# MSU-dcypherlab/mfgp-coverage

Measured on NVIDIA B200. Metric: GP posterior mean+var + coverage step, grid-points/s (coverage iterations/s = 1000/ms_per_step), higher is better.
Workload: dtype f64

## Files before the change

### mfgp-coverage_b200/csrc/common.cuh

```cuda
#pragma once
#include <cstdint>
#include <cstdio>
#include <cuda_runtime.h>

#include "../../include/mfgp_b200.h"

namespace mfgp {

void set_last_error(const char* what, cudaError_t e);

#define MFGP_CUDA_CHECK(expr)                                   \
    do {                                                        \
        cudaError_t _e = (expr);                                \
        if (_e != cudaSuccess) {                                \
            ::mfgp::set_last_error(#expr, _e);                  \
            return MFGP_ERR_CUDA;                               \
        }                                                       \
    } while (0)

void count_launch();
#define MFGP_LAUNCH_CHECK()                  \
    do {                                     \
        ::mfgp::count_launch();              \
        MFGP_CUDA_CHECK(cudaGetLastError()); \
    } while (0)

__device__ __forceinline__ void dmma884(double& c0, double& c1, double a, double b) {
    asm volatile("mma.sync.aligned.m8n8k4.row.col.f64.f64.f64.f64 {%0,%1}, {%2}, {%3}, {%0,%1};\n"
                 : "+d"(c0), "+d"(c1)
                 : "d"(a), "d"(b));
}

__device__ __forceinline__ void cp_async16(void* smem_dst, const void* gmem_src, bool valid) {
    unsigned s = static_cast<unsigned>(__cvta_generic_to_shared(smem_dst));
    int bytes = valid ? 16 : 0;
    asm volatile("cp.async.cg.shared.global [%0], [%1], 16, %2;\n" ::"r"(s), "l"(gmem_src), "r"(bytes));
}
__device__ __forceinline__ void cp_async_commit() { asm volatile("cp.async.commit_group;\n" ::); }
template <int N>
__device__ __forceinline__ void cp_async_wait() {
    asm volatile("cp.async.wait_group %0;\n" ::"n"(N));
}

__device__ __forceinline__ double rbf_scaled(double ax, double ay, double bx, double by, double scale) {
    double d0 = ax - bx, d1 = ay - by;
    double q = __dadd_rn(__dmul_rn(d0, d0), __dmul_rn(d1, d1));
    return scale * exp(-0.5 * q);
}

struct DevParams {
    double s_L, inv_unused, s_H, rho, rho2, noise_L, noise_H, mean_L, mean_H, jitter, l_L, l_H, k0;
    int multi;
};

inline DevParams make_dev_params(const mfgp_params& p) {
    DevParams d;
    d.s_L = p.multi ? p.s_L : 0.0;
    d.inv_unused = 0.0;
    d.s_H = p.s_H;
    d.rho = p.multi ? p.rho : 1.0;
    d.rho2 = d.rho * d.rho;
    d.noise_L = p.noise_L;
    d.noise_H = p.noise_H;
    d.mean_L = p.mean_L;
    d.mean_H = p.mean_H;
    d.jitter = p.jitter;
// ... 9 lines not shown
```

### mfgp-coverage_b200/csrc/gp_fit.cu

```cuda
#include "common.cuh"
#include "gemm_f64.cuh"
#include <cstdlib>
#include <cstring>

namespace mfgp {

__global__ void scaled_coords_kernel(const double* __restrict__ Xt, int N, int npad, DevParams p, double* __restrict__ Tt) {
    const int i = blockIdx.x * blockDim.x + threadIdx.x;
    if (i >= npad) return;
    double4 t = make_double4(0.0, 0.0, 0.0, 0.0);
    if (i < N) {
        const double xi = Xt[2 * i], yi = Xt[2 * i + 1];
        t = make_double4(xi / p.l_L, yi / p.l_L, xi / p.l_H, yi / p.l_H);
    }
    reinterpret_cast<double4*>(Tt)[i] = t;
}

__global__ void build_train_cov_kernel(const double* __restrict__ Xt, int NL, int NH, DevParams p, double* __restrict__ K,
                                       int npad, int64_t ld, const double* __restrict__ Tt, int row_begin) {
    const int j = blockIdx.x * blockDim.x + threadIdx.x;
    const int i = row_begin + blockIdx.y * blockDim.y + threadIdx.y;
    const int N = NL + NH;
    if (i >= npad || j >= npad) return;
    if (j >= ((i >> 6) + 1) * 64) return;
// ... 22 lines not shown
                const double kH = rbf_scaled(a.z, a.w, b.z, b.w, p.s_H);
                v = __dadd_rn(__dmul_rn(p.rho2, kL), kH);
                if (i == j) v = v + p.noise_H;
            }
        } else {
            v = rbf_scaled(a.z, a.w, b.z, b.w, p.s_H);
            if (i == j) v = v + p.noise_H;
        }
        if (i == j) v = v + p.jitter;
    }
    K[(int64_t)i * ld + j] = v;
}

constexpr int PB = 64;
constexpr int PLD = PB + 1;

struct PotrfScratch {
    double2 colAB[2][PB], rowAB[2][PB];
    double piv[3][PB / 2];
    double fin[3][PB / 2];
    int bad;
};

template <int BS>
__device__ __forceinline__ void potrf_diag_body(const double* src, int64_t lds, double* A, int64_t ld,
                                                double* __restrict__ Winv, int64_t ldw, int32_t* __restrict__ info, int col0,
                                                PotrfScratch* sc, double* Lsm = nullptr, double* Wsm = nullptr, int lds_out = 0) {
    constexpr int NB = BS / 16;
    double2 (*colAB)[PB] = sc->colAB;
    double2 (*rowAB)[PB] = sc->rowAB;
    double (*piv)[PB / 2] = sc->piv;
    double (*fin)[PB / 2] = sc->fin;
    int& bad = sc->bad;
    const int tid = threadIdx.x;
    const int ti = tid >> 4, tc = tid & 15;
    if (tid == 0) bad = 0;
    double s[NB][NB], m[NB][NB];
#pragma unroll
    for (int a = 0; a < NB; a++)
#pragma unroll
        for (int b = 0; b < NB; b++) {
            const int r = ti + 16 * a, c = tc + 16 * b;
            s[a][b] = (c <= r) ? src[(int64_t)r * lds + c] : 0.0;
            m[a][b] = (r == c) ? 1.0 : 0.0;
        }
#pragma unroll
    for (int jb = 0; jb < NB; jb++) {
#pragma unroll 1
        for (int jp = 0; jp < 8; jp++) {
            const int k = jb * 8 + jp, j0 = 2 * k, j1 = j0 + 1, jj0 = 2 * jp, buf = k & 1;
            if ((tc & 14) == jj0) {
                double* dst = reinterpret_cast<double*>(colAB[buf]) + (tc & 1);
#pragma unroll
                for (int a = 0; a < NB; a++) dst[2 * (ti + 16 * a)] = s[a][jb];
            }
            if ((ti & 14) == jj0) {
                double* dst = reinterpret_cast<double*>(rowAB[buf]) + (ti & 1);
#pragma unroll
                for (int b = 0; b < NB; b++) dst[2 * (tc + 16 * b)] = m[jb][b];
            }
            __syncthreads();
            const double2* col = colAB[buf];
            const double2* row = rowAB[buf];
            double pa = col[j0].x;
            const double2 p1 = col[j1];
            double pb = p1.x, pc = p1.y;
            double det = fma(pa, pc, -(pb * pb));
            if (!(pa > 0.0) || !(det > 0.0)) {
                if (tid == 0 && !bad) {
                    bad = 1;
                    atomicCAS(info, 0, col0 + ((pa > 0.0) ? j1 : j0) + 1);
                }
                pa = 1.0; pb = 0.0; pc = 1.0; det = 1.0;
            }
            if (tid == 0) { piv[0][k] = pa; piv[1][k] = pb; piv[2][k] = pc; }
            const double idet = 1.0 / det;
            const double qa = pc * idet, qb = -pb * idet, qc = pa * idet;
            double t1[NB], t2[NB];
#pragma unroll
            for (int a = 0; a < NB; a++) {
                if (a < jb) continue;
                const double2 x = col[ti + 16 * a];
                t1[a] = fma(qa, x.x, qb * x.y);
                t2[a] = fma(qb, x.x, qc * x.y);
// ... 2 lines not shown
            for (int b = 0; b < NB; b++) {
                if (b < jb) continue;
                const double2 y = col[tc + 16 * b];
                const bool live = tc + 16 * b > j1;
#pragma unroll
                for (int a = 0; a < NB; a++) {
                    if (a < b) continue;
                    if (live) s[a][b] = fma(-t1[a], y.x, fma(-t2[a], y.y, s[a][b]));
                }
            }
#pragma unroll
            for (int b = 0; b < NB; b++) {
                if (b > jb) continue;
                const double2 z = row[tc + 16 * b];
#pragma unroll
                for (int a = 0; a < NB; a++) {
                    if (a < jb) continue;
                    const bool live = ti + 16 * a > j1;
                    if (live) m[a][b] = fma(-t1[a], z.x, fma(-t2[a], z.y, m[a][b]));
                }
            }
        }
    }
    __syncthreads();
    if (tid < BS / 2) {
        const double a = piv[0][tid], b = piv[1][tid], c = piv[2][tid];
        const double r1 = rsqrt(a);
        const double g = b * r1 * r1;
        fin[0][tid] = r1;
        fin[1][tid] = rsqrt(fma(-g, b, c));
        fin[2][tid] = g;
    }
    __syncthreads();
    const bool failed = bad != 0;
#pragma unroll
    for (int a = 0; a < NB; a++)
#pragma unroll
        for (int b = 0; b < NB; b++) {
            const int r = ti + 16 * a, c = tc + 16 * b;
            const double v = s[a][b], w = m[a][b];
            const double vp = __shfl_up_sync(0xffffffffu, v, 1);
            const double wp = __shfl_up_sync(0xffffffffu, w, 16);
            const int kc = c >> 1, kr = r >> 1;
            const double lv = (c & 1) ? (v - fin[2][kc] * vp) * fin[1][kc] : v * fin[0][kc];
            const double wv = (r & 1) ? (w - fin[2][kr] * wp) * fin[1][kr] : w * fin[0][kr];
            const double lo = failed ? ((r == c) ? 1.0 : 0.0) : ((c <= r) ? lv : 0.0);
            const double wo = failed ? ((r == c) ? 1.0 : 0.0) : ((c <= r) ? wv : 0.0);
            if (c <= r) A[(int64_t)r * ld + c] = lo;
            if (Winv != nullptr) Winv[(int64_t)r * ldw + c] = wo;
            if (Lsm != nullptr) Lsm[r * lds_out + c] = lo;
            if (Wsm != nullptr) Wsm[r * lds_out + c] = wo;
        }
}

__global__ void __launch_bounds__(256, 1) potrf_diag_kernel(double* __restrict__ A, int64_t ld, double* __restrict__ Winv,
                                                         int64_t ldw, int32_t* __restrict__ info, int jblk) {
    __shared__ __align__(16) PotrfScratch scratch;
    potrf_diag_body<PB>(A, ld, A, ld, Winv, ldw, info, jblk * PB, &scratch);
}

constexpr int DF_K = 32;
constexpr int DF_LDA = DF_K + 4;
constexpr int DF_LDT = PB + 4;
constexpr int DF_STAGE = PB * DF_LDA;
constexpr int DF_TILE = PB * DF_LDT;
constexpr int DF_NSTAGE = 3;
constexpr int DF_SMEM_DOUBLES = DF_NSTAGE * 2 * DF_STAGE;
constexpr int DF_THREADS = 256;

struct DfArgs {
    double* K; int64_t ld;
    double* W; int64_t ldw;
    double* Bm; int64_t ldb;
    int nb, nr;
    int32_t* info;
    int* flagsL;
    int* flagsY;
    int* ctrl;
    int* pause;
    int total;
    double* M; int64_t ldm;
    int* flagsM;
    int mg, m_full, m_tiles, m_total, m_lead;
    long long spin_limit;
    long long* trace;
    int chain_la;
};

__host__ __device__ __forceinline__ void df_group_rows(int gi, int nb, int mg, int m_full, int& kb, int& ke) {
    if (gi < m_full) { kb = gi * mg; ke = kb + mg; return; }
    kb = m_full * mg;
// ... 13 lines not shown

__device__ __forceinline__ void df_stamp(long long* trace, int task, int k) {
    if (trace != nullptr && threadIdx.x == 0) {
        unsigned long long t;
        asm volatile("mov.u64 %0, %%globaltimer;\n" : "=l"(t));
        trace[task * 16 + k] = (long long)t;
        trace[task * 16 + 8 + k] = clock64();
    }
}

__device__ __forceinline__ int df_ld_acquire(const int* p) {
    int v;
    asm volatile("ld.acquire.gpu.global.s32 %0, [%1];\n" : "=r"(v) : "l"(p) : "memory");
    return v;
}
__device__ __forceinline__ int df_ld_relaxed(const int* p) {
    int v;
    asm volatile("ld.relaxed.gpu.global.s32 %0, [%1];\n" : "=r"(v) : "l"(p) : "memory");
    return v;
}
__device__ __forceinline__ void df_st_release(int* p, int v) {
    asm volatile("st.release.gpu.global.s32 [%0], %1;\n" ::"l"(p), "r"(v) : "memory");
}
__device__ __forceinline__ void df_st_relaxed(int* p, int v) {
    asm volatile("st.relaxed.gpu.global.s32 [%0], %1;\n" ::"l"(p), "r"(v) : "memory");
}
__device__ __forceinline__ bool df_wait(const int* f, int* ctrl, int32_t* info, long long limit) {
    int ok = 1;
    if ((threadIdx.x & 31) == 0) {
        if (!df_ld_relaxed(f)) {
            const long long t0 = clock64();
            while (!df_ld_relaxed(f)) {
                __nanosleep(32);
                if (clock64() - t0 > limit) { atomicExch(ctrl + 1, 1); atomicExch(info, -1); }
                if (*reinterpret_cast<volatile int*>(ctrl + 1)) { ok = 0; break; }
            }
        }
        (void)df_ld_acquire(f);
    }
    ok = __shfl_sync(0xffffffffu, ok, 0);
    __syncwarp();
    return ok != 0;
}

__global__ void __launch_bounds__(DF_THREADS, 2) chol_dataflow_kernel(DfArgs g) {
    extern __shared__ __align__(16) double df_smem[];
    __shared__ int task[4];
    __shared__ int ready_s[4];
    const int tid = threadIdx.x, lane = tid & 31, warp = tid >> 5;
    const int wm = (warp >> 1) * 8, wn = (warp & 1) * 8;
    const int gq = lane >> 2, tq = lane & 3;
    double* As0 = df_smem;
    double* Bs0 = df_smem + DF_NSTAGE * DF_STAGE;
    unsigned smid;
    asm volatile("mov.u32 %0, %%smid;\n" : "=r"(smid));
    int* my_pause = g.pause + smid;
#ifdef MFGP_DF_ACCOUNTING
    long long t_wait = 0, t_loop = 0, t_begin = clock64(), t_mark = 0;
    int n_tasks = 0;
    const bool tracing = g.trace != nullptr;
#else
    long long t_wait = 0, t_loop = 0, t_begin = 0, t_mark = 0;
    int n_tasks = 0;
    constexpr bool tracing = false;
#endif
    int held_m = -1;
    int dec_c = 0, dec_dnext = 1, dec_base = 1;

    for (;;) {
// ... 506 lines not shown
int side_for_current_device(SideStream** out) {
    int dev = 0;
    MFGP_CUDA_CHECK(cudaGetDevice(&dev));
    if (dev < 0 || dev >= 16) return MFGP_ERR_INVALID;
    SideStream& s = g_side[dev];
    if (!s.st) {
        int least = 0, greatest = 0;
        MFGP_CUDA_CHECK(cudaDeviceGetStreamPriorityRange(&least, &greatest));
        MFGP_CUDA_CHECK(cudaStreamCreateWithPriority(&s.st, cudaStreamNonBlocking, greatest));
        for (int i = 0; i < 2; i++) {
            MFGP_CUDA_CHECK(cudaEventCreateWithFlags(&s.ev_potrf[i], cudaEventDisableTiming));
            MFGP_CUDA_CHECK(cudaEventCreateWithFlags(&s.ev_trsm[i], cudaEventDisableTiming));
        }
        MFGP_CUDA_CHECK(cudaEventCreateWithFlags(&s.ev_begin, cudaEventDisableTiming));
        MFGP_CUDA_CHECK(cudaEventCreateWithFlags(&s.ev_end, cudaEventDisableTiming));
        s.device = dev;
    }
    *out = &s;
    return MFGP_OK;
}
}

namespace {
struct DfScratch {
    long long* trace = nullptr;
    int trace_nb = 0;
    int trace_grid = 0;
    int sms = 0;
};
DfScratch g_df[16];

bool use_panel_chain() {
    static const int v = [] {
        const char* e = getenv("MFGP_CHOL");
        return (e && std::strcmp(e, "chain") == 0) ? 1 : 0;
    }();
    return v != 0;
}

int chol_dataflow(double* K, int64_t npad, int64_t ld, double* W, int64_t ldw, int32_t* info, double* Bm, int64_t ldb, int64_t R,
                  double* M, int64_t ldm, int* scratch, cudaStream_t st) {
    int dev = 0;
    MFGP_CUDA_CHECK(cudaGetDevice(&dev));
    if (dev < 0 || dev >= 16 || !scratch) return MFGP_ERR_INVALID;
    DfScratch& sc = g_df[dev];
    const int nb = (int)(npad / PB), nr = (int)(R / PB);
    const int64_t need = df_scratch_ints(npad, R, M != nullptr);
    if (!sc.sms) MFGP_CUDA_CHECK(cudaDeviceGetAttribute(&sc.sms, cudaDevAttrMultiProcessorCount, dev));
    MFGP_CUDA_CHECK(cudaMemsetAsync(scratch, 0, need * sizeof(int), st));
    MFGP_CUDA_CHECK(cudaMemsetAsync(info, 0, sizeof(int32_t), st));
    DfArgs a{};
    a.K = K; a.ld = ld; a.W = W; a.ldw = ldw; a.Bm = Bm; a.ldb = ldb; a.nb = nb; a.nr = nr; a.info = info;
    a.ctrl = scratch; a.pause = scratch + DF_CTRL_INTS; a.flagsL = a.pause + 1024; a.flagsY = a.flagsL + (int64_t)nb * nb;
    a.total = nb + (nb - 1) * (nb - 2) / 2 + nb * nr;
    if (M != nullptr && nr > 0) {
        static const int mg_env = [] { const char* e = getenv("MFGP_DF_MG"); return e ? atoi(e) : 8; }();
        static const int lead_env = [] { const char* e = getenv("MFGP_DF_MLEAD"); return e ? atoi(e) : 32; }();
        a.M = M; a.ldm = ldm; a.flagsM = a.flagsY + (int64_t)nb * nr;
        a.mg = mg_env < DF_MIN_MG ? DF_MIN_MG : mg_env;
        a.m_tiles = nr * (nr + 1) / 2;
        a.m_total = df_gram_groups(nb, a.mg, a.m_full) * a.m_tiles;
        a.m_lead = lead_env;
    }
    static const bool want_trace = [] { const char* e = getenv("MFGP_DF_TRACE"); return e && atoi(e) != 0; }();
    if (want_trace) {
        if (!sc.trace) MFGP_CUDA_CHECK(cudaMalloc(&sc.trace, 1024 * 24 * sizeof(long long)));
        MFGP_CUDA_CHECK(cudaMemsetAsync(sc.trace, 0, 1024 * 24 * sizeof(long long), st));
        a.trace = nb <= 1024 ? sc.trace : nullptr;
        sc.trace_nb = nb;
    }
    static const int chain_la = [] { const char* e = getenv("MFGP_DF_CHAIN_LA"); return e ? atoi(e) : 5; }();
    a.chain_la = chain_la;
    a.spin_limit = 4000000000LL;
    constexpr int smem = DF_SMEM_DOUBLES * sizeof(double);
    static const int occ = [] { const char* e = getenv("MFGP_DF_OCC"); return e ? atoi(e) : 2; }();
    MFGP_CUDA_CHECK(cudaFuncSetAttribute(chol_dataflow_kernel, cudaFuncAttributeMaxDynamicSharedMemorySize, smem));
    int grid = (occ < 1 ? 1 : occ) * sc.sms;
    if (grid > a.total + a.m_total) grid = a.total + a.m_total;
    sc.trace_grid = grid < 1024 ? grid : 1024;
    chol_dataflow_kernel<<<grid, DF_THREADS, smem, st>>>(a);
    MFGP_LAUNCH_CHECK();
    return MFGP_OK;
}
}

extern "C" int64_t mfgp_debug_chol_trace(int64_t* out, int64_t max_tasks) {
    int dev = 0;
    if (cudaGetDevice(&dev) != cudaSuccess || dev < 0 || dev >= 16) return 0;
    DfScratch& sc = g_df[dev];
    if (!sc.trace || !out) return 0;
    if (max_tasks < 0) {
        if (cudaMemcpy(out, sc.trace + 1024 * 16, 1024 * 8 * sizeof(long long), cudaMemcpyDeviceToHost) != cudaSuccess) return 0;
        return sc.trace_grid;
    }
    int64_t n = sc.trace_nb < max_tasks ? sc.trace_nb : max_tasks;
    if (cudaMemcpy(out, sc.trace, n * 16 * sizeof(long long), cudaMemcpyDeviceToHost) != cudaSuccess) return 0;
    return n;
}

extern "C" int mfgp_cholesky(double* K, int64_t npad, int64_t ld, double* W, int64_t ldw, int32_t* info, void* work,
                             void* stream) {
    if (!K || !info || npad <= 0 || npad % MFGP_TILE || ld < npad) return MFGP_ERR_INVALID;
    if (!W && !work) return MFGP_ERR_INVALID;
// ... 256 lines not shown
```

### mfgp-coverage_b200/csrc/gp_posterior.cu

```cuda
#include <cuda.h>

#include "common.cuh"

namespace mfgp {

constexpr int P_BM = 512;
constexpr int P_BN = 32;
constexpr int P_BK = 16;
constexpr int P_STAGES = 3;
constexpr int P_CONSUMER_WARPS = 8;
constexpr int P_PRODUCER_WARPS = 4;
constexpr int P_THREADS = (P_CONSUMER_WARPS + P_PRODUCER_WARPS) * 32;
constexpr int P_MI = 8;
constexpr int P_NI = 4;
constexpr int P_PLD = P_BK + 4;
constexpr int P_W_STAGE_BYTES = P_BM * P_BK * 8;
constexpr int P_PSI_STAGE_BYTES = P_BN * P_PLD * 8;
constexpr int P_SMEM_BYTES = P_STAGES * (P_W_STAGE_BYTES + P_PSI_STAGE_BYTES) + P_BN * 4 * 8 +
                             P_CONSUMER_WARPS * P_BN * 2 * 8 + 2 * P_STAGES * 8 + 1024 ;

struct PostArgs {
    const double* Xs; int64_t G;
    const double* TLx; const double* TLy; const double* THx; const double* THy;
    int64_t ldt; int64_t g_lo; int ny;
    const double* Tt; int NL, NH;
    int npad;
    const double* z;
    double* mu; double* var; double* qout;
    double* Vc; int64_t ldv;
    int remap_cols;
    int row_lo;
    DevParams p;
};

__device__ __forceinline__ uint32_t smem_u32(const void* p) { return static_cast<uint32_t>(__cvta_generic_to_shared(p)); }
__device__ __forceinline__ void mbar_init(uint32_t bar, uint32_t count) {
    asm volatile("mbarrier.init.shared::cta.b64 [%0], %1;\n" ::"r"(bar), "r"(count));
}
__device__ __forceinline__ void mbar_arrive(uint32_t bar) {
    asm volatile("mbarrier.arrive.shared::cta.b64 _, [%0];\n" ::"r"(bar) : "memory");
}
__device__ __forceinline__ void mbar_expect_tx(uint32_t bar, uint32_t bytes) {
    asm volatile("mbarrier.expect_tx.relaxed.cta.shared::cta.b64 [%0], %1;\n" ::"r"(bar), "r"(bytes) : "memory");
}
__device__ __forceinline__ void mbar_wait(uint32_t bar, uint32_t parity) {
    uint32_t done;
    do {
        asm volatile(
            "{\n .reg .pred p;\n mbarrier.try_wait.parity.shared::cta.b64 p, [%1], %2;\n selp.u32 %0, 1, 0, p;\n}\n"
            : "=r"(done)
            : "r"(bar), "r"(parity)
            : "memory");
    } while (!done);
}
__device__ __forceinline__ void tma_load_2d(uint32_t dst, const CUtensorMap* map, int c0, int c1, uint32_t bar) {
    asm volatile(
        "cp.async.bulk.tensor.2d.shared::cluster.global.mbarrier::complete_tx::bytes [%0], [%1, {%2, %3}], [%4];\n" ::"r"(dst),
        "l"(map), "r"(c0), "r"(c1), "r"(bar)
        : "memory");
}
template <int R>
__device__ __forceinline__ void reg_alloc() { asm volatile("setmaxnreg.inc.sync.aligned.u32 %0;\n" ::"n"(R)); }
template <int R>
__device__ __forceinline__ void reg_dealloc() { asm volatile("setmaxnreg.dec.sync.aligned.u32 %0;\n" ::"n"(R)); }

__device__ __forceinline__ int row_perm(int g) { return ((g & 3) << 1) | (g >> 2); }

template <bool GRID>
__global__ void __launch_bounds__(P_THREADS, 1)
posterior_kernel(const __grid_constant__ CUtensorMap wmap, PostArgs a) {
    extern __shared__ uint8_t smem_raw[];
    uint8_t* smem = reinterpret_cast<uint8_t*>((reinterpret_cast<uintptr_t>(smem_raw) + 1023) & ~uintptr_t(1023));
    uint8_t* Wst = smem;
    double* Pst = reinterpret_cast<double*>(smem + P_STAGES * P_W_STAGE_BYTES);
    double* xs = Pst + P_STAGES * P_BN * P_PLD;
    double* colacc = xs + P_BN * 4;
    uint64_t* bars = reinterpret_cast<uint64_t*>(colacc + P_CONSUMER_WARPS * P_BN * 2);
    const uint32_t full0 = smem_u32(bars), empty0 = smem_u32(bars + P_STAGES);

    const int tid = threadIdx.x, lane = tid & 31, warp = tid >> 5;
    const int64_t g0 = (GRID && a.remap_cols > 0)
                           ? (int64_t)(blockIdx.x % a.remap_cols) * a.ny + (int64_t)(blockIdx.x / a.remap_cols) * P_BN
// ... 484 lines not shown
    }
}

__global__ void grid_tables_kernel(const double* __restrict__ u, int nu, int axis, const double* __restrict__ Tt, int NL, int NH,
                                   int npad, DevParams p, double* __restrict__ TL, double* __restrict__ TH, int64_t ldt) {
    const int n = blockIdx.x * blockDim.x + threadIdx.x;
    const int iu = blockIdx.y;
    if (n >= npad || iu >= nu) return;
    const int N = NL + NH;
    double vl = 0.0, vh = 0.0;
    if (n < N) {
        const double4 t = reinterpret_cast<const double4*>(Tt)[n];
        const double uv = u[iu];
        const double dl = uv / p.l_L - (axis == 0 ? t.x : t.y);
        const double dh = uv / p.l_H - (axis == 0 ? t.z : t.w);
        const bool lo = n < NL;
        if (p.multi) vl = exp(-0.5 * (dl * dl)) * (axis == 0 ? (lo ? p.rho * p.s_L : p.rho2 * p.s_L) : 1.0);
        if (!lo) vh = exp(-0.5 * (dh * dh)) * (axis == 0 ? p.s_H : 1.0);
    }
    TL[(int64_t)iu * ldt + n] = vl;
    TH[(int64_t)iu * ldt + n] = vh;
}

typedef CUresult (*EncodeTiledFn)(CUtensorMap*, CUtensorMapDataType, cuuint32_t, void*, const cuuint64_t*, const cuuint64_t*,
                                  const cuuint32_t*, const cuuint32_t*, CUtensorMapInterleave, CUtensorMapSwizzle,
                                  CUtensorMapL2promotion, CUtensorMapFloatOOBfill);

static int make_w_tensor_map(CUtensorMap* map, const double* W, int64_t npad, int64_t ldw, int box_rows = P_BM / 2) {
    static EncodeTiledFn encode = nullptr;
    if (!encode) {
        void* fn = nullptr;
        cudaDriverEntryPointQueryResult qres;
        MFGP_CUDA_CHECK(cudaGetDriverEntryPoint("cuTensorMapEncodeTiled", &fn, cudaEnableDefault, &qres));
        if (qres != cudaDriverEntryPointSuccess || !fn) {
            set_last_error("cuTensorMapEncodeTiled entry point unavailable", cudaErrorUnknown);
            return MFGP_ERR_CUDA;
        }
        encode = reinterpret_cast<EncodeTiledFn>(fn);
    }
    const cuuint64_t gdim[2] = {(cuuint64_t)npad, (cuuint64_t)npad};
    const cuuint64_t gstride[1] = {(cuuint64_t)ldw * sizeof(double)};
    const cuuint32_t box[2] = {(cuuint32_t)P_BK, (cuuint32_t)box_rows};
    const cuuint32_t estr[2] = {1, 1};
    const CUresult r = encode(map, CU_TENSOR_MAP_DATA_TYPE_FLOAT64, 2, const_cast<double*>(W), gdim, gstride, box, estr,
                              CU_TENSOR_MAP_INTERLEAVE_NONE, CU_TENSOR_MAP_SWIZZLE_128B, CU_TENSOR_MAP_L2_PROMOTION_L2_256B,
                              CU_TENSOR_MAP_FLOAT_OOB_FILL_NONE);
    if (r != CUDA_SUCCESS) {
        set_last_error("cuTensorMapEncodeTiled failed", cudaErrorInvalidValue);
        return MFGP_ERR_CUDA;
    }
    return MFGP_OK;
}

}

using namespace mfgp;

static int posterior_common(PostArgs& a, bool grid, const double* W, int64_t npad, int64_t ldw, const mfgp_params* p_host,
                            cudaStream_t st) {
    const DevParams dp = make_dev_params(*p_host);
    a.p = dp;
    const int64_t N = (int64_t)a.NL + a.NH;
    if (N == 0) {
        posterior_prior_kernel<<<(unsigned)((a.G + 255) / 256), 256, 0, st>>>(a.G, dp.mean_H, dp.k0, a.mu, a.var, a.qout);
        MFGP_LAUNCH_CHECK();
        return MFGP_OK;
    }
    if (!W || !a.z || npad < N || npad % MFGP_TILE || ldw < npad) return MFGP_ERR_INVALID;
    if ((reinterpret_cast<uintptr_t>(W) & 15) || (ldw & 1)) return MFGP_ERR_INVALID;
    if (!p_host->multi && a.NL != 0) return MFGP_ERR_INVALID;
    if (a.Vc && a.ldv < a.G) return MFGP_ERR_INVALID;
    if (a.row_lo < 0 || a.row_lo >= N) return MFGP_ERR_INVALID;
    CUtensorMap wmap;
    a.npad = (int)npad;
// ... 99 lines not shown
```

Before: 446.0 million.

## Add warp-specialized TMA producer to dataflow Cholesky kernel for large problems

Adds a dedicated producer warp to the dataflow Cholesky kernel. It polls dependency flags and issues TMA bulk tensor loads into a multi-stage mbarrier pipeline, replacing cp.async loads issued by the compute threads. Compute-only barriers become named bar.sync on 256 threads so the producer is excluded, and publishing now adds async-proxy fences. The old cp.async kernel is kept for matrices below a tile-count threshold, and tensor maps are cached per buffer. The change adds extra control complexity, a register cap, and new paths that could deadlock.

```diff
diff --git a/mfgp-coverage_b200/csrc/common.cuh b/mfgp-coverage_b200/csrc/common.cuh
--- a/mfgp-coverage_b200/csrc/common.cuh
+++ b/mfgp-coverage_b200/csrc/common.cuh
@@ -1,6 +1,7 @@
 #pragma once
 #include <cstdint>
 #include <cstdio>
+#include <cuda.h>
 #include <cuda_runtime.h>
 
 #include "../../include/mfgp_b200.h"
@@ -42,6 +43,63 @@
     asm volatile("cp.async.wait_group %0;\n" ::"n"(N));
 }
 
+__device__ __forceinline__ uint32_t smem_u32(const void* p) { return static_cast<uint32_t>(__cvta_generic_to_shared(p)); }
+__device__ __forceinline__ void mbar_init(uint32_t bar, uint32_t count) {
+    asm volatile("mbarrier.init.shared::cta.b64 [%0], %1;\n" ::"r"(bar), "r"(count));
+}
+__device__ __forceinline__ void mbar_arrive(uint32_t bar) {
+    asm volatile("mbarrier.arrive.shared::cta.b64 _, [%0];\n" ::"r"(bar) : "memory");
+}
+__device__ __forceinline__ void mbar_arrive_expect_tx(uint32_t bar, uint32_t bytes) {
+    asm volatile("mbarrier.arrive.expect_tx.shared::cta.b64 _, [%0], %1;\n" ::"r"(bar), "r"(bytes) : "memory");
+}
+__device__ __forceinline__ void mbar_wait(uint32_t bar, uint32_t parity) {
+    uint32_t done;
+    do {
+        asm volatile(
+            "{\n .reg .pred p;\n mbarrier.try_wait.parity.shared::cta.b64 p, [%1], %2;\n selp.u32 %0, 1, 0, p;\n}\n"
+            : "=r"(done)
+            : "r"(bar), "r"(parity)
+            : "memory");
+    } while (!done);
+}
+__device__ __forceinline__ void tma_load_2d(uint32_t dst, const CUtensorMap* map, int c0, int c1, uint32_t bar) {
+    asm volatile(
+        "cp.async.bulk.tensor.2d.shared::cluster.global.mbarrier::complete_tx::bytes [%0], [%1, {%2, %3}], [%4];\n" ::"r"(dst),
+        "l"(map), "r"(c0), "r"(c1), "r"(bar)
+        : "memory");
+}
+
+typedef CUresult (*EncodeTiledFn)(CUtensorMap*, CUtensorMapDataType, cuuint32_t, void*, const cuuint64_t*, const cuuint64_t*,
+                                  const cuuint32_t*, const cuuint32_t*, CUtensorMapInterleave, CUtensorMapSwizzle,
+                                  CUtensorMapL2promotion, CUtensorMapFloatOOBfill);
+inline int make_tensor_map_2d(CUtensorMap* map, const double* base, int64_t rows, int64_t cols, int64_t ld, int box_cols,
+                              int box_rows, CUtensorMapSwizzle swizzle) {
+    static EncodeTiledFn encode = nullptr;
+    if (!encode) {
+        void* fn = nullptr;
+        cudaDriverEntryPointQueryResult qres;
+        MFGP_CUDA_CHECK(cudaGetDriverEntryPoint("cuTensorMapEncodeTiled", &fn, cudaEnableDefault, &qres));
+        if (qres != cudaDriverEntryPointSuccess || !fn) {
+            set_last_error("cuTensorMapEncodeTiled entry point unavailable", cudaErrorUnknown);
+            return MFGP_ERR_CUDA;
+        }
+        encode = reinterpret_cast<EncodeTiledFn>(fn);
+    }
+    const cuuint64_t gdim[2] = {(cuuint64_t)cols, (cuuint64_t)rows};
+    const cuuint64_t gstride[1] = {(cuuint64_t)ld * sizeof(double)};
+    const cuuint32_t box[2] = {(cuuint32_t)box_cols, (cuuint32_t)box_rows};
+    const cuuint32_t estr[2] = {1, 1};
+    const CUresult r = encode(map, CU_TENSOR_MAP_DATA_TYPE_FLOAT64, 2, const_cast<double*>(base), gdim, gstride, box, estr,
+                              CU_TENSOR_MAP_INTERLEAVE_NONE, swizzle, CU_TENSOR_MAP_L2_PROMOTION_L2_256B,
+                              CU_TENSOR_MAP_FLOAT_OOB_FILL_NONE);
+    if (r != CUDA_SUCCESS) {
+        set_last_error("cuTensorMapEncodeTiled failed", cudaErrorInvalidValue);
+        return MFGP_ERR_CUDA;
+    }
+    return MFGP_OK;
+}
+
 __device__ __forceinline__ double rbf_scaled(double ax, double ay, double bx, double by, double scale) {
     double d0 = ax - bx, d1 = ay - by;
     double q = __dadd_rn(__dmul_rn(d0, d0), __dmul_rn(d1, d1));
diff --git a/mfgp-coverage_b200/csrc/gp_fit.cu b/mfgp-coverage_b200/csrc/gp_fit.cu
--- a/mfgp-coverage_b200/csrc/gp_fit.cu
+++ b/mfgp-coverage_b200/csrc/gp_fit.cu
@@ -68,6 +68,8 @@
     int bad;
 };
 
+__device__ __forceinline__ void tile_bar() { asm volatile("bar.sync 1, 256;\n" ::: "memory"); }
+
 template <int BS>
 __device__ __forceinline__ void potrf_diag_body(const double* src, int64_t lds, double* A, int64_t ld,
                                                 double* __restrict__ Winv, int64_t ldw, int32_t* __restrict__ info, int col0,
@@ -105,7 +107,7 @@
 #pragma unroll
                 for (int b = 0; b < NB; b++) dst[2 * (tc + 16 * b)] = m[jb][b];
             }
-            __syncthreads();
+            tile_bar();
             const double2* col = colAB[buf];
             const double2* row = rowAB[buf];
             double pa = col[j0].x;
@@ -154,7 +156,7 @@
             }
         }
     }
-    __syncthreads();
+    tile_bar();
     if (tid < BS / 2) {
         const double a = piv[0][tid], b = piv[1][tid], c = piv[2][tid];
         const double r1 = rsqrt(a);
@@ -163,7 +165,7 @@
         fin[1][tid] = rsqrt(fma(-g, b, c));
         fin[2][tid] = g;
     }
-    __syncthreads();
+    tile_bar();
     const bool failed = bad != 0;
 #pragma unroll
     for (int a = 0; a < NB; a++)
@@ -198,7 +200,13 @@
 constexpr int DF_TILE = PB * DF_LDT;
 constexpr int DF_NSTAGE = 3;
 constexpr int DF_SMEM_DOUBLES = DF_NSTAGE * 2 * DF_STAGE;
+constexpr int DF_SMEM_BYTES = DF_SMEM_DOUBLES * 8 + 128;
 constexpr int DF_THREADS = 256;
+constexpr int DF_CTA_THREADS = DF_THREADS + 32;
+constexpr uint32_t DF_MK_BYTES = PB * DF_LDA * 8;
+constexpr uint32_t DF_KN_BYTES = DF_K * DF_LDT * 8;
+constexpr uint32_t DF_TILE_BYTES = PB * DF_LDT * 8;
+constexpr int DF_TMA_MIN_NB = 33;
 
 struct DfArgs {
     double* K; int64_t ld;
@@ -258,6 +266,10 @@
 __device__ __forceinline__ void df_st_release(int* p, int v) {
     asm volatile("st.release.gpu.global.s32 [%0], %1;\n" ::"l"(p), "r"(v) : "memory");
 }
+__device__ __forceinline__ void df_publish(int* flag) {
+    asm volatile("fence.proxy.async.global;\n" ::: "memory");
+    df_st_release(flag, 1);
+}
 __device__ __forceinline__ void df_st_relaxed(int* p, int v) {
     asm volatile("st.relaxed.gpu.global.s32 [%0], %1;\n" ::"l"(p), "r"(v) : "memory");
 }
@@ -279,8 +291,495 @@
     return ok != 0;
 }
 
-__global__ void __launch_bounds__(DF_THREADS, 2) chol_dataflow_kernel(DfArgs g) {
-    extern __shared__ __align__(16) double df_smem[];
+struct DfOut {
+    double* Ct; int64_t ldc;
+    double* Cd;
+    int* flag;
+};
+__device__ __forceinline__ DfOut df_out(const DfArgs& g, const int* task) {
+    const int kind = task[0], idx = task[2], tj = task[3];
+    const bool rhs = kind == 1, chain = kind == 2, gram = kind == 3;
+    const int c = chain ? idx - 1 : (gram ? 0 : task[1]), cc = c > 0 ? c : 0;
+    const int i = rhs ? c : idx;
+    DfOut o;
+    o.Ct = gram ? g.M + (int64_t)idx * PB * g.ldm + (int64_t)tj * PB
+                : (rhs ? g.Bm + (int64_t)c * PB * g.ldb + (int64_t)idx * PB : g.K + (int64_t)i * PB * g.ld + (int64_t)cc * PB);
+    o.ldc = gram ? g.ldm : (rhs ? g.ldb : g.ld);
+    o.Cd = g.K + (int64_t)(chain ? idx : 0) * PB * (g.ld + 1);
+    o.flag = gram ? g.flagsM + (int64_t)task[1] * g.m_tiles + idx * (idx + 1) / 2 + tj
+                  : (rhs ? g.flagsY + (int64_t)c * g.nr + idx : g.flagsL + (int64_t)i * g.nb + cc);
+    return o;
+}
+
+__device__ __forceinline__ int df_poll_tiles(const int* fa, int fas, const int* fb, int fbs, int kt0, int nk, int* ctrl, int32_t* info,
+                                          long long limit) {
+    const int lane = threadIdx.x & 31, j = lane & 15, kt = kt0 + j;
+    const int* f = lane < 16 ? fa + (int64_t)kt * fas : fb + (int64_t)kt * fbs;
+    long long t0 = 0;
+    for (int spin = 0;; spin++) {
+        const int v = (kt < nk && (spin == 0 || j == 0)) ? df_ld_relaxed(f) : 0;
+        const unsigned m = __ballot_sync(0xffffffffu, v != 0);
+        const unsigned both = m & (m >> 16) & 0xffffu;
+        const int n = __ffs(~both) - 1;
+        if (n > 0) {
+            if (j < n) (void)df_ld_acquire(f);
+            __syncwarp();
+            return kt0 + n - 1;
+        }
+        int stop = 0;
+        if (lane == 0) {
+            if (spin == 0) t0 = clock64();
+            else if (clock64() - t0 > limit) { atomicExch(ctrl + 1, 1); atomicExch(info, -1); }
+            stop = *reinterpret_cast<volatile int*>(ctrl + 1);
+        }
+        if (__shfl_sync(0xffffffffu, stop, 0)) return -1;
+        __nanosleep(32);
+    }
+}
+
+__global__ void __maxnreg__(112)
+chol_dataflow_kernel(const __grid_constant__ CUtensorMap kmap, const __grid_constant__ CUtensorMap bmap,
+                     const __grid_constant__ CUtensorMap wmap, DfArgs g) {
+    extern __shared__ __align__(128) uint8_t df_smem_raw[];
+    double* df_smem = reinterpret_cast<double*>(df_smem_raw + ((128u - (smem_u32(df_smem_raw) & 127u)) & 127u));
+    __shared__ int task[6];
+    __shared__ int ready_s[4];
+    __shared__ int dec_s[6];
+    __shared__ int abort_s;
+    __shared__ __align__(8) unsigned long long df_bars[2 * DF_NSTAGE + 1];
+    const int tid = threadIdx.x, lane = tid & 31, warp = tid >> 5;
+    const bool producer = warp == DF_THREADS / 32;
+    const uint32_t bar_full = smem_u32(&df_bars[0]), bar_empty = smem_u32(&df_bars[DF_NSTAGE]);
+    const uint32_t bar_w = smem_u32(&df_bars[2 * DF_NSTAGE]);
+    if (tid == 0) {
+        for (int q = 0; q < DF_NSTAGE; q++) { mbar_init(bar_full + 8 * q, 1); mbar_init(bar_empty + 8 * q, DF_THREADS / 32); }
+        mbar_init(bar_w, 1);
+        abort_s = 0;
+        dec_s[0] = -1; dec_s[1] = 0; dec_s[2] = 1; dec_s[3] = 1; dec_s[4] = 0; dec_s[5] = 0;
+        asm volatile("fence.mbarrier_init.release.cluster;\n" ::: "memory");
+    }
+    const int wm = (warp >> 1) * 8, wn = (warp & 1) * 8;
+    const int gq = lane >> 2, tq = lane & 3;
+    double* As0 = df_smem;
+    double* Bs0 = df_smem + DF_NSTAGE * DF_STAGE;
+    auto my_pause = [&]() {
+        unsigned smid;
+        asm volatile("mov.u32 %0, %%smid;\n" : "=r"(smid));
+        return g.pause + smid;
+    };
+#ifdef MFGP_DF_ACCOUNTING
+    long long t_wait = 0, t_loop = 0, t_begin = clock64(), t_mark = 0;
+    int n_tasks = 0;
+    const bool tracing = g.trace != nullptr;
+#else
+    long long t_wait = 0, t_loop = 0, t_begin = 0, t_mark = 0;
+    int n_tasks = 0;
+    constexpr bool tracing = false;
+#endif
+    int& held_m = dec_s[0];
+    int& dec_c = dec_s[1];
+    int& dec_dnext = dec_s[2];
+    int& dec_base = dec_s[3];
+
+    for (;;) {
+        if (!producer) asm volatile("fence.proxy.async.shared::cta;\n" ::: "memory");
+        __syncthreads();
+        if (producer && lane == 0) {
+            int c = 0, kind = -1, idx = 0, aux = 0;
+            int t = -1;
+            if (g.M == nullptr) {
+                t = atomicAdd(g.ctrl, 1);
+            } else {
+                for (;;) {
+                    const int front = df_ld_relaxed(g.ctrl + 3), drawn = df_ld_relaxed(g.ctrl + 4);
+                    const bool crit_left = df_ld_relaxed(g.ctrl) < g.total;
+                    auto runnable = [&](int tm) {
+                        int kb_, ke_;
+                        df_group_rows(tm / g.m_tiles, g.nb, g.mg, g.m_full, kb_, ke_);
+                        const int last_row = ke_ - 1;
+                        return !crit_left || (drawn > last_row && last_row + 2 <= front);
+                    };
+                    if (held_m < 0) {
+                        const int tm = df_ld_relaxed(g.ctrl + 2);
+                        if (tm < g.m_total && runnable(tm) && (!crit_left || drawn - front >= g.m_lead)) {
+                            const int got = atomicAdd(g.ctrl + 2, 1);
+                            if (got < g.m_total) held_m = got;
+                        }
+                    }
+                    if (held_m >= 0 && runnable(held_m)) {
+                        kind = 3; c = held_m / g.m_tiles; idx = held_m % g.m_tiles;
+                        int ti = 0;
+                        while ((ti + 1) * (ti + 2) / 2 <= idx) ti++;
+                        aux = idx - ti * (ti + 1) / 2;
+                        idx = ti;
+                        held_m = -1;
+                        break;
+                    }
+                    if (crit_left) {
+                        t = atomicAdd(g.ctrl, 1);
+                        if (t < g.total) break;
+                        t = -1;
+                        continue;
+                    }
+                    if (held_m < 0 && df_ld_relaxed(g.ctrl + 2) >= g.m_total) break;
+                }
+            }
+            if (t == 0) {
+                kind = 2; idx = 0;
+            } else if (t > 0 && t < g.total) {
+                for (;;) {
+                    int nchain = 0;
+                    while (dec_dnext + nchain < g.nb) {
+                        const int d = dec_dnext + nchain;
+                        const int place = max(0, d - 1 - (g.chain_la > 0 ? d / g.chain_la : 0));
+                        if (place != dec_c) break;
+                        nchain++;
+                    }
+                    const int ntile = g.nb - dec_c - 2 > 0 ? g.nb - dec_c - 2 : 0;
+                    const int n = nchain + ntile + g.nr;
+                    if (t < dec_base + n) {
+                        const int tl = t - dec_base;
+                        c = dec_c;
+                        if (tl < nchain) { kind = 2; idx = dec_dnext + tl; }
+                        else if (tl < nchain + ntile) { kind = 0; idx = c + 2 + (tl - nchain); }
+                        else { kind = 1; idx = tl - nchain - ntile; }
+                        break;
+                    }
+                    dec_base += n; dec_c++; dec_dnext += nchain;
+                }
+                if (g.M != nullptr) atomicMax(g.ctrl + 4, c);
+            }
+            task[3] = aux;
+            task[0] = kind; task[1] = c; task[2] = idx;
+            task[4] = dec_s[4]; task[5] = dec_s[5];
+        }
+        __syncthreads();
+        const int kind = task[0], idx = task[2];
+        if (kind < 0) {
+            if (tracing && tid == 0) {
+                unsigned long long tg;
+                asm volatile("mov.u64 %0, %%globaltimer;\n" : "=l"(tg));
+                long long* o = g.trace + 1024 * 16 + (int64_t)blockIdx.x * 8;
+                o[0] = t_wait; o[1] = t_loop; o[2] = clock64() - t_begin; o[3] = n_tasks; o[4] = (long long)tg; o[5] = my_pause() - g.pause;
+            }
+            return;
+        }
+        n_tasks++;
+        const bool rhs = kind == 1, chain = kind == 2, gram = kind == 3;
+        const bool bkn = rhs || gram;
+        const int c = chain ? idx - 1 : (gram ? 0 : task[1]);
+        const int i = rhs ? c : idx;
+        const int gi = gram ? task[1] : 0, tj = task[3];
+        int kb = 0, ke_g = 0;
+        if (gram) df_group_rows(gi, g.nb, g.mg, g.m_full, kb, ke_g);
+        const int nk = gram ? ke_g - kb : (chain ? (idx > 0 ? idx - 1 : 0) : c);
+        const int* fa = gram ? g.flagsY + (int64_t)kb * g.nr + idx : g.flagsL + (int64_t)i * g.nb;
+        const int* fb = gram ? g.flagsY + (int64_t)kb * g.nr + tj
+                             : (rhs ? g.flagsY + idx : g.flagsL + (int64_t)(c > 0 ? c : 0) * g.nb);
+        const int fas = gram ? g.nr : 1, fbs = bkn ? g.nr : 1;
+        const int nslab = nk * (PB / DF_K);
+        if (gram && gi > 0) {
+            if (tracing) t_mark = clock64();
+            if (producer) {
+                const bool w = df_wait(df_out(g, task).flag - g.m_tiles, g.ctrl, g.info, g.spin_limit);
+                if (lane == 0) ready_s[2] = w ? 1 : 0;
+            }
+            __syncthreads();
+            if (tracing) t_wait += clock64() - t_mark;
+            if (ready_s[2] == 0) return;
+        }
+
+        if (producer) {
+            const CUtensorMap* amap = gram ? &bmap : &kmap;
+            const CUtensorMap* bsrc = bkn ? &bmap : &kmap;
+            const int a_col = gram ? idx * PB : 0, a_row = gram ? kb * PB : i * PB;
+            const int b_col = gram ? tj * PB : (rhs ? idx * PB : 0);
+            const int b_row = gram ? kb * PB : (rhs ? 0 : (c > 0 ? c : 0) * PB);
+            const uint32_t bytes = (gram ? DF_KN_BYTES : DF_MK_BYTES) + (bkn ? DF_KN_BYTES : DF_MK_BYTES);
+            int ready_kt = -1, paused = 0;
+            for (int s = 0; s < nslab; s++) {
+                const bool fresh = (s >> 1) > ready_kt;
+                if (fresh) {
+                    const int r = df_poll_tiles(fa, fas, fb, fbs, s >> 1, nk, g.ctrl, g.info, g.spin_limit);
+                    if (r < 0) {
+                        if (lane == 0) abort_s = 1;
+                        ready_kt = nk;
+                    } else {
+                        ready_kt = r;
+                    }
+                }
+                if (lane == 0) {
+                    const unsigned gs = (unsigned)task[4] + s;
+                    const int slot = gs % DF_NSTAGE;
+                    while (paused && df_ld_relaxed(my_pause()) && !*reinterpret_cast<volatile int*>(g.ctrl + 1)) __nanosleep(200);
+                    if (gs >= DF_NSTAGE) mbar_wait(bar_empty + 8 * slot, ((gs / DF_NSTAGE) + 1) & 1);
+                    if (fresh) asm volatile("fence.proxy.async.global;\n" ::: "memory");
+                    const uint32_t fbar = bar_full + 8 * slot;
+                    mbar_arrive_expect_tx(fbar, bytes);
+                    const int k0 = s * DF_K;
+                    tma_load_2d(smem_u32(As0 + slot * DF_STAGE), amap, gram ? a_col : k0, gram ? a_row + k0 : a_row, fbar);
+                    tma_load_2d(smem_u32(Bs0 + slot * DF_STAGE), bsrc, bkn ? b_col : k0, bkn ? b_row + k0 : b_row, fbar);
+                    paused = df_ld_relaxed(my_pause());
+                }
+            }
+            if (lane == 0) dec_s[4] += nslab;
+            __syncthreads();
+            if (abort_s) return;
+            if (gram || (chain && idx == 0)) continue;
+            const bool w = df_wait(g.flagsL + (int64_t)c * g.nb + c, g.ctrl, g.info, g.spin_limit);
+            if (lane == 0) {
+                ready_s[3] = w ? 1 : 0;
+                dec_s[5]++;
+                if (w) {
+                    if (chain) df_st_relaxed(my_pause(), 1);
+                    asm volatile("fence.proxy.async.global;\n" ::: "memory");
+                    mbar_arrive_expect_tx(bar_w, DF_TILE_BYTES);
+                    tma_load_2d(smem_u32(df_smem + DF_TILE), &wmap, c * PB, c * PB, bar_w);
+                } else {
+                    mbar_arrive(bar_w);
+                }
+            }
+            if (!w) return;
+            continue;
+        }
+
+        const bool has_tile = gram ? gi > 0 : !(chain && idx == 0);
+        double acc[2][4][2], acc2[2][4][2];
+        const DfOut in = df_out(g, task);
+#pragma unroll
+        for (int x = 0; x < 2; x++)
+#pragma unroll
+            for (int y = 0; y < 4; y++) {
+                const int r = wm + x * 32 + gq, cc = wn + y * 16 + tq * 2;
+                double2 v = make_double2(0.0, 0.0), d = make_double2(0.0, 0.0);
+                if (has_tile) v = *reinterpret_cast<const double2*>(in.Ct + (int64_t)r * in.ldc + cc);
+                if (chain) d = *reinterpret_cast<const double2*>(in.Cd + (int64_t)r * g.ld + cc);
+                acc[x][y][0] = gram ? v.x : -v.x; acc[x][y][1] = gram ? v.y : -v.y;
+                acc2[x][y][0] = -d.x; acc2[x][y][1] = -d.y;
+            }
+
+        auto compute = [&](int slot) {
+            const double* As = As0 + slot * DF_STAGE;
+            const double* Bs = Bs0 + slot * DF_STAGE;
+#pragma unroll
+            for (int kk = 0; kk < DF_K; kk += 4) {
+                double a[2], b[4];
+#pragma unroll
+                for (int x = 0; x < 2; x++)
+                    a[x] = gram ? As[(kk + tq) * DF_LDT + wm + x * 32 + gq] : As[(wm + x * 32 + gq) * DF_LDA + kk + tq];
+#pragma unroll
+                for (int y = 0; y < 4; y++)
+                    b[y] = bkn ? Bs[(kk + tq) * DF_LDT + wn + y * 16 + gq] : Bs[(wn + y * 16 + gq) * DF_LDA + kk + tq];
+#pragma unroll
+                for (int x = 0; x < 2; x++)
+#pragma unroll
+                    for (int y = 0; y < 4; y++) dmma884(acc[x][y][0], acc[x][y][1], a[x], b[y]);
+                if (chain) {
+#pragma unroll
+                    for (int y = 0; y < 4; y++) b[y] = As[(wn + y * 16 + gq) * DF_LDA + kk + tq];
+#pragma unroll
+                    for (int x = 0; x < 2; x++)
+#pragma unroll
+                        for (int y = 0; y < 4; y++)
+                            if (wn + y * 16 < wm + x * 32 + 8) dmma884(acc2[x][y][0], acc2[x][y][1], a[x], b[y]);
+                }
+            }
+        };
+        const long long t_loop0 = tracing ? clock64() : 0;
+        const unsigned gs0 = task[4];
+        for (int s = 0; s < nslab; s++) {
+            const unsigned gs = gs0 + s;
+            const int slot = gs % DF_NSTAGE;
+            if (tracing) t_mark = clock64();
+            mbar_wait(bar_full + 8 * slot, (gs / DF_NSTAGE) & 1);
+            if (tracing) t_wait += clock64() - t_mark;
+            compute(slot);
+            __syncwarp();
+            if (lane == 0) mbar_arrive(bar_empty + 8 * slot);
+        }
+        __syncthreads();
+        if (abort_s) return;
+
+        if (tracing) t_loop += clock64() - t_loop0;
+        if (chain) df_stamp(g.trace, idx, 0);
+        double* Xs = df_smem;
+        double* Ws = df_smem + DF_TILE;
+        double* Ls = df_smem + 2 * DF_TILE;
+        const DfOut out = df_out(g, task);
+        double* const Ct = out.Ct;
+        const int64_t ldc = out.ldc;
+        double* const Cd = out.Cd;
+        if (gram) {
+#pragma unroll
+            for (int x = 0; x < 2; x++)
+#pragma unroll
+                for (int y = 0; y < 4; y++) {
+                    const int r = wm + x * 32 + gq, cc = wn + y * 16 + tq * 2;
+                    double2 v;
+                    v.x = acc[x][y][0]; v.y = acc[x][y][1];
+                    *reinterpret_cast<double2*>(Ct + (int64_t)r * ldc + cc) = v;
+                }
+        } else if (!(chain && idx == 0)) {
+#pragma unroll
+            for (int x = 0; x < 2; x++)
+#pragma unroll
+                for (int y = 0; y < 4; y++) {
+                    const int r = wm + x * 32 + gq, cc = wn + y * 16 + tq * 2;
+                    Xs[r * DF_LDT + cc] = -acc[x][y][0];
+                    Xs[r * DF_LDT + cc + 1] = -acc[x][y][1];
+                    acc[x][y][0] = acc[x][y][1] = 0.0;
+                }
+            if (tracing) t_mark = clock64();
+            tile_bar();
+            if (chain) df_stamp(g.trace, idx, 1);
+            mbar_wait(bar_w, task[5] & 1);
+            if (tracing) t_wait += clock64() - t_mark;
+            if (ready_s[3] == 0) return;
+            if (chain) df_stamp(g.trace, idx, 2);
+#pragma unroll 4
+            for (int kk = 0; kk < PB; kk += 4) {
+                double a[2], b[4];
+                if (!rhs) {
+#pragma unroll
+                    for (int x = 0; x < 2; x++) a[x] = Xs[(wm + x * 32 + gq) * DF_LDT + kk + tq];
+#pragma unroll
+                    for (int y = 0; y < 4; y++) b[y] = (kk < wn + y * 16 + 8) ? Ws[(wn + y * 16 + gq) * DF_LDT + kk + tq] : 0.0;
+#pragma unroll
+                    for (int x = 0; x < 2; x++)
+#pragma unroll
+                        for (int y = 0; y < 4; y++)
+                            if (kk < wn + y * 16 + 8) dmma884(acc[x][y][0], acc[x][y][1], a[x], b[y]);
+                    continue;
+                } else {
+#pragma unroll
+                    for (int x = 0; x < 2; x++) a[x] = Ws[(wm + x * 32 + gq) * DF_LDT + kk + tq];
+#pragma unroll
+                    for (int y = 0; y < 4; y++) b[y] = Xs[(kk + tq) * DF_LDT + wn + y * 16 + gq];
+                }
+#pragma unroll
+                for (int x = 0; x < 2; x++)
+#pragma unroll
+                    for (int y = 0; y < 4; y++) dmma884(acc[x][y][0], acc[x][y][1], a[x], b[y]);
+            }
+#pragma unroll
+            for (int x = 0; x < 2; x++)
+#pragma unroll
+                for (int y = 0; y < 4; y++) {
+                    const int r = wm + x * 32 + gq, cc = wn + y * 16 + tq * 2;
+                    double2 v;
+                    v.x = acc[x][y][0]; v.y = acc[x][y][1];
+                    *reinterpret_cast<double2*>(Ct + (int64_t)r * ldc + cc) = v;
+                    if (chain) { Ls[r * DF_LDT + cc] = v.x; Ls[r * DF_LDT + cc + 1] = v.y; }
+                }
+        }
+        if (chain) {
+            double* Wd = g.W + (int64_t)idx * PB * (g.ldw + 1);
+            df_stamp(g.trace, idx, 3);
+            if (idx > 0) {
+                tile_bar();
+#pragma unroll 4
+                for (int kk = 0; kk < PB; kk += 4) {
+                    double a[2], b[4];
+#pragma unroll
+                    for (int x = 0; x < 2; x++) a[x] = Ls[(wm + x * 32 + gq) * DF_LDT + kk + tq];
+#pragma unroll
+                    for (int y = 0; y < 4; y++) b[y] = Ls[(wn + y * 16 + gq) * DF_LDT + kk + tq];
+#pragma unroll
+                    for (int x = 0; x < 2; x++)
+#pragma unroll
+                        for (int y = 0; y < 4; y++)
+                            if (wn + y * 16 < wm + x * 32 + 8) dmma884(acc2[x][y][0], acc2[x][y][1], a[x], b[y]);
+                }
+            }
+#pragma unroll
+            for (int x = 0; x < 2; x++)
+#pragma unroll
+                for (int y = 0; y < 4; y++) {
+                    const int r = wm + x * 32 + gq, cc = wn + y * 16 + tq * 2;
+                    Xs[r * DF_LDT + cc] = -acc2[x][y][0];
+                    Xs[r * DF_LDT + cc + 1] = -acc2[x][y][1];
+                }
+            if (idx > 0) {
+                tile_bar();
+                if (tid == 0) df_publish(out.flag);
+            } else {
+                tile_bar();
+            }
+            df_stamp(g.trace, idx, 4);
+            {
+                PotrfScratch* sc = reinterpret_cast<PotrfScratch*>(Ws);
+                constexpr int H = PB / 2, LO = DF_LDT;
+                double* L11s = Ls;
+                double* W11s = Ls + H;
+                double* L21s = Ls + H * LO;
+                double* Tsm = Ls + H * LO + H;
+                double* W22s = Xs;
+                const int m0 = (warp >> 1) * 8, n0 = (warp & 1) * 16;
+                auto mm32 = [&](const double* A, const double* B, bool b_nk, double (&c)[2][2]) {
+                    c[0][0] = c[0][1] = c[1][0] = c[1][1] = 0.0;
+#pragma unroll
+                    for (int kk = 0; kk < H; kk += 4) {
+                        const double av = A[(m0 + gq) * LO + kk + tq];
+#pragma unroll
+                        for (int j = 0; j < 2; j++) {
+                            const double bv = b_nk ? B[(n0 + 8 * j + gq) * LO + kk + tq] : B[(kk + tq) * LO + n0 + 8 * j + gq];
+                            dmma884(c[j][0], c[j][1], av, bv);
+                        }
+                    }
+                };
+                double c[2][2];
+                potrf_diag_body<H>(Xs, LO, Cd, g.ld, Wd, g.ldw, g.info, idx * PB, sc, L11s, W11s, LO);
+                tile_bar();
+                mm32(Xs + H * LO, W11s, true, c);
+#pragma unroll
+                for (int j = 0; j < 2; j++) {
+                    const int r = m0 + gq, cc = n0 + 8 * j + tq * 2;
+                    *reinterpret_cast<double2*>(Cd + (int64_t)(H + r) * g.ld + cc) = make_double2(c[j][0], c[j][1]);
+                    L21s[r * LO + cc] = c[j][0]; L21s[r * LO + cc + 1] = c[j][1];
+                }
+                tile_bar();
+                mm32(L21s, L21s, true, c);
+#pragma unroll
+                for (int j = 0; j < 2; j++) {
+                    const int r = m0 + gq, cc = n0 + 8 * j + tq * 2;
+                    Xs[(H + r) * LO + H + cc] -= c[j][0]; Xs[(H + r) * LO + H + cc + 1] -= c[j][1];
+                }
+                tile_bar();
+                potrf_diag_body<H>(Xs + H * LO + H, LO, Cd + (int64_t)H * g.ld + H, g.ld, Wd + (int64_t)H * g.ldw + H, g.ldw, g.info,
+                                   idx * PB + H, sc, nullptr, W22s, LO);
+                tile_bar();
+                mm32(L21s, W11s, false, c);
+#pragma unroll
+                for (int j = 0; j < 2; j++) {
+                    const int r = m0 + gq, cc = n0 + 8 * j + tq * 2;
+                    Tsm[r * LO + cc] = c[j][0]; Tsm[r * LO + cc + 1] = c[j][1];
+                }
+                tile_bar();
+                mm32(W22s, Tsm, false, c);
+#pragma unroll
+                for (int j = 0; j < 2; j++) {
+                    const int r = m0 + gq, cc = n0 + 8 * j + tq * 2;
+                    *reinterpret_cast<double2*>(Wd + (int64_t)(H + r) * g.ldw + cc) = make_double2(-c[j][0], -c[j][1]);
+                    *reinterpret_cast<double2*>(Wd + (int64_t)r * g.ldw + H + cc) = make_double2(0.0, 0.0);
+                }
+            }
+            df_stamp(g.trace, idx, 5);
+        }
+        tile_bar();
+        if (tid == 0) {
+            df_publish(chain ? g.flagsL + (int64_t)idx * g.nb + idx : out.flag);
+            if (chain) {
+                df_st_relaxed(my_pause(), 0);
+                if (g.M != nullptr) atomicMax(g.ctrl + 3, idx + 1);
+            }
+        }
+        if (chain) df_stamp(g.trace, idx, 6);
+    }
+}
+
+__global__ void __launch_bounds__(DF_THREADS, 2) chol_dataflow_cpasync_kernel(DfArgs g) {
+    extern __shared__ __align__(16) double df_smem_c[];
+    double* df_smem = df_smem_c;
     __shared__ int task[4];
     __shared__ int ready_s[4];
     const int tid = threadIdx.x, lane = tid & 31, warp = tid >> 5;
@@ -833,11 +1332,26 @@
 }
 
 namespace {
+struct DfMap {
+    const double* base = nullptr;
+    int64_t rows = 0, cols = 0, ld = 0;
+    CUtensorMap map;
+};
+int df_cached_map(DfMap& m, const double* base, int64_t rows, int64_t cols, int64_t ld, int box_cols, int box_rows) {
+    if (m.base == base && m.rows == rows && m.cols == cols && m.ld == ld) return MFGP_OK;
+    m.base = nullptr;
+    const int rc = make_tensor_map_2d(&m.map, base, rows, cols, ld, box_cols, box_rows, CU_TENSOR_MAP_SWIZZLE_NONE);
+    if (rc) return rc;
+    m.base = base; m.rows = rows; m.cols = cols; m.ld = ld;
+    return MFGP_OK;
+}
+
 struct DfScratch {
     long long* trace = nullptr;
     int trace_nb = 0;
     int trace_grid = 0;
     int sms = 0;
+    DfMap kmap, bmap, wmap;
 };
 DfScratch g_df[16];
 
@@ -883,13 +1397,26 @@
     static const int chain_la = [] { const char* e = getenv("MFGP_DF_CHAIN_LA"); return e ? atoi(e) : 5; }();
     a.chain_la = chain_la;
     a.spin_limit = 4000000000LL;
-    constexpr int smem = DF_SMEM_DOUBLES * sizeof(double);
+    auto aligned = [](const void* p, int64_t l) { return (reinterpret_cast<uintptr_t>(p) & 15) == 0 && (l & 1) == 0; };
+    if (!aligned(K, ld) || !aligned(W, ldw) || (nr > 0 && !aligned(Bm, ldb))) return MFGP_ERR_INVALID;
     static const int occ = [] { const char* e = getenv("MFGP_DF_OCC"); return e ? atoi(e) : 2; }();
-    MFGP_CUDA_CHECK(cudaFuncSetAttribute(chol_dataflow_kernel, cudaFuncAttributeMaxDynamicSharedMemorySize, smem));
     int grid = (occ < 1 ? 1 : occ) * sc.sms;
     if (grid > a.total + a.m_total) grid = a.total + a.m_total;
     sc.trace_grid = grid < 1024 ? grid : 1024;
-    chol_dataflow_kernel<<<grid, DF_THREADS, smem, st>>>(a);
+    if (nb < DF_TMA_MIN_NB) {
+        constexpr int smem_c = DF_SMEM_DOUBLES * sizeof(double);
+        MFGP_CUDA_CHECK(cudaFuncSetAttribute(chol_dataflow_cpasync_kernel, cudaFuncAttributeMaxDynamicSharedMemorySize, smem_c));
+        chol_dataflow_cpasync_kernel<<<grid, DF_THREADS, smem_c, st>>>(a);
+        MFGP_LAUNCH_CHECK();
+        return MFGP_OK;
+    }
+    int rc = df_cached_map(sc.kmap, K, npad, npad, ld, DF_LDA, PB);
+    if (!rc) rc = df_cached_map(sc.wmap, W, npad, npad, ldw, DF_LDT, PB);
+    if (!rc && nr > 0) rc = df_cached_map(sc.bmap, Bm, npad, R, ldb, DF_LDT, DF_K);
+    if (rc) return rc;
+    constexpr int smem = DF_SMEM_BYTES;
+    MFGP_CUDA_CHECK(cudaFuncSetAttribute(chol_dataflow_kernel, cudaFuncAttributeMaxDynamicSharedMemorySize, smem));
+    chol_dataflow_kernel<<<grid, DF_CTA_THREADS, smem, st>>>(sc.kmap.map, nr > 0 ? sc.bmap.map : sc.kmap.map, sc.wmap.map, a);
     MFGP_LAUNCH_CHECK();
     return MFGP_OK;
 }
diff --git a/mfgp-coverage_b200/csrc/gp_posterior.cu b/mfgp-coverage_b200/csrc/gp_posterior.cu
--- a/mfgp-coverage_b200/csrc/gp_posterior.cu
+++ b/mfgp-coverage_b200/csrc/gp_posterior.cu
@@ -33,31 +33,8 @@
     DevParams p;
 };
 
-__device__ __forceinline__ uint32_t smem_u32(const void* p) { return static_cast<uint32_t>(__cvta_generic_to_shared(p)); }
-__device__ __forceinline__ void mbar_init(uint32_t bar, uint32_t count) {
-    asm volatile("mbarrier.init.shared::cta.b64 [%0], %1;\n" ::"r"(bar), "r"(count));
-}
-__device__ __forceinline__ void mbar_arrive(uint32_t bar) {
-    asm volatile("mbarrier.arrive.shared::cta.b64 _, [%0];\n" ::"r"(bar) : "memory");
-}
 __device__ __forceinline__ void mbar_expect_tx(uint32_t bar, uint32_t bytes) {
     asm volatile("mbarrier.expect_tx.relaxed.cta.shared::cta.b64 [%0], %1;\n" ::"r"(bar), "r"(bytes) : "memory");
-}
-__device__ __forceinline__ void mbar_wait(uint32_t bar, uint32_t parity) {
-    uint32_t done;
-    do {
-        asm volatile(
-            "{\n .reg .pred p;\n mbarrier.try_wait.parity.shared::cta.b64 p, [%1], %2;\n selp.u32 %0, 1, 0, p;\n}\n"
-            : "=r"(done)
-            : "r"(bar), "r"(parity)
-            : "memory");
-    } while (!done);
-}
-__device__ __forceinline__ void tma_load_2d(uint32_t dst, const CUtensorMap* map, int c0, int c1, uint32_t bar) {
-    asm volatile(
-        "cp.async.bulk.tensor.2d.shared::cluster.global.mbarrier::complete_tx::bytes [%0], [%1, {%2, %3}], [%4];\n" ::"r"(dst),
-        "l"(map), "r"(c0), "r"(c1), "r"(bar)
-        : "memory");
 }
 template <int R>
 __device__ __forceinline__ void reg_alloc() { asm volatile("setmaxnreg.inc.sync.aligned.u32 %0;\n" ::"n"(R)); }
@@ -588,34 +565,8 @@
     TH[(int64_t)iu * ldt + n] = vh;
 }
 
-typedef CUresult (*EncodeTiledFn)(CUtensorMap*, CUtensorMapDataType, cuuint32_t, void*, const cuuint64_t*, const cuuint64_t*,
-                                  const cuuint32_t*, const cuuint32_t*, CUtensorMapInterleave, CUtensorMapSwizzle,
-                                  CUtensorMapL2promotion, CUtensorMapFloatOOBfill);
-
 static int make_w_tensor_map(CUtensorMap* map, const double* W, int64_t npad, int64_t ldw, int box_rows = P_BM / 2) {
-    static EncodeTiledFn encode = nullptr;
-    if (!encode) {
-        void* fn = nullptr;
-        cudaDriverEntryPointQueryResult qres;
-        MFGP_CUDA_CHECK(cudaGetDriverEntryPoint("cuTensorMapEncodeTiled", &fn, cudaEnableDefault, &qres));
-        if (qres != cudaDriverEntryPointSuccess || !fn) {
-            set_last_error("cuTensorMapEncodeTiled entry point unavailable", cudaErrorUnknown);
-            return MFGP_ERR_CUDA;
-        }
-        encode = reinterpret_cast<EncodeTiledFn>(fn);
-    }
-    const cuuint64_t gdim[2] = {(cuuint64_t)npad, (cuuint64_t)npad};
-    const cuuint64_t gstride[1] = {(cuuint64_t)ldw * sizeof(double)};
-    const cuuint32_t box[2] = {(cuuint32_t)P_BK, (cuuint32_t)box_rows};
-    const cuuint32_t estr[2] = {1, 1};
-    const CUresult r = encode(map, CU_TENSOR_MAP_DATA_TYPE_FLOAT64, 2, const_cast<double*>(W), gdim, gstride, box, estr,
-                              CU_TENSOR_MAP_INTERLEAVE_NONE, CU_TENSOR_MAP_SWIZZLE_128B, CU_TENSOR_MAP_L2_PROMOTION_L2_256B,
-                              CU_TENSOR_MAP_FLOAT_OOB_FILL_NONE);
-    if (r != CUDA_SUCCESS) {
-        set_last_error("cuTensorMapEncodeTiled failed", cudaErrorInvalidValue);
-        return MFGP_ERR_CUDA;
-    }
-    return MFGP_OK;
+    return make_tensor_map_2d(map, W, npad, npad, ldw, P_BK, box_rows, CU_TENSOR_MAP_SWIZZLE_128B);
 }
 
 }
```

New measurement: 467.8 million, median of 6. +4.9%, better.
